# gortiz/pinot

Measured on AMD Instinct MI355X. Metric: rows scanned/sec + achieved HBM GB/s, filter+group-by query, 1/2/4/8 GPUs, higher is better.
Workload: dtype int32/int64/f64

## Files before the change

### include/pinot_amd.h

```cpp
#ifndef PINOT_AMD_H
#define PINOT_AMD_H

#include <stddef.h>
#include <stdint.h>

#ifdef __cplusplus
extern "C" {
#endif

#define PINOT_AMD_ABI_VERSION 1

#define PINOT_AMD_OK 0
#define PINOT_AMD_EINVAL (-1)
#define PINOT_AMD_EUNSUPPORTED (-2)
#define PINOT_AMD_EHIP (-3)
#define PINOT_AMD_ENOMEM (-4)
#define PINOT_AMD_EOVERFLOW (-5)

enum pinot_amd_data_type { PINOT_AMD_INT = 0, PINOT_AMD_LONG = 1, PINOT_AMD_FLOAT = 2, PINOT_AMD_DOUBLE = 3,
                           PINOT_AMD_STRING = 4 };

enum pinot_amd_fwd_encoding {
  PINOT_AMD_FWD_FIXED_BIT = 0,
  PINOT_AMD_FWD_RAW = 1,
// ... 121 lines not shown
int pinot_amd_result_accumulators(pinot_amd_result* r, int32_t* h_num_slots, int64_t* h_num_key_slots,
                                  void** h_slot_ptrs, int32_t* h_slot_ops);
int pinot_amd_result_export_groups(pinot_amd_result* r, uint64_t* d_keys, uint64_t* d_acc, int64_t cap,
                                   int32_t* h_key_words, int32_t* h_num_acc, int64_t* h_num_groups, void* stream);
int pinot_amd_result_merge_groups(pinot_amd_result* r, const uint64_t* d_keys, const uint64_t* d_acc, int64_t n,
                                  void* stream);
int pinot_amd_result_fetch_distinct_values(pinot_amd_result* r, int32_t agg_index, int64_t cap, int64_t* h_offsets,
                                           int64_t* h_values, int64_t* h_num_values);
int pinot_amd_result_fetch_value_counts(pinot_amd_result* r, int32_t agg_index, int64_t cap, int64_t* h_offsets,
                                        int64_t* h_values, int64_t* h_counts, int64_t* h_num_values);
const char* pinot_amd_result_distinct_string(pinot_amd_result* r, int32_t agg_index, int64_t id);

const char* pinot_amd_result_kernel_info(pinot_amd_result* r);
int pinot_amd_result_algorithmic_bytes(pinot_amd_result* r, double* h_bytes);
const char* pinot_amd_result_packed_info(pinot_amd_result* r);
const char* pinot_amd_result_plan_timing(pinot_amd_result* r);
int pinot_amd_result_last_kernel_ms(pinot_amd_result* r, double* h_ms);

#ifdef __cplusplus
}
#endif
#endif
```

### pinot_amd/_lib.py

```python
from __future__ import annotations

import ctypes as C
import os

try:
    import torch
except Exception:
    torch = None

HERE = os.path.dirname(os.path.abspath(__file__))
LIB_PATH = os.path.join(HERE, "libpinot_amd.so")


class PinotAmdError(RuntimeError):
    pass


class ColumnSpec(C.Structure):
    _fields_ = [
        ("name", C.c_char_p), ("stored_type", C.c_int32), ("encoding", C.c_int32), ("cardinality", C.c_int32),
        ("bits_per_element", C.c_int32), ("h_fwd", C.c_void_p), ("fwd_size", C.c_size_t),
        ("h_dictionary", C.c_void_p), ("dictionary_size", C.c_size_t), ("h_inverted", C.c_void_p),
        ("inverted_size", C.c_size_t),
    ]
# ... 65 lines not shown
    "pinot_amd_result_accumulators": (C.c_int, [_P, C.POINTER(C.c_int32), _I64P, _PP, C.POINTER(C.c_int32)]),
    "pinot_amd_result_check_word": (C.c_int, [_P, _PP]),
    "pinot_amd_selfcheck_failures": (C.c_int64, []),
    "pinot_amd_result_export_groups": (C.c_int, [_P, _P, _P, C.c_int64, C.POINTER(C.c_int32), C.POINTER(C.c_int32),
                                                 _I64P, _P]),
    "pinot_amd_result_merge_groups": (C.c_int, [_P, _P, _P, C.c_int64, _P]),
    "pinot_amd_result_plan_timing": (C.c_char_p, [_P]),
    "pinot_amd_query_set_result_limit": (C.c_int, [_P, C.c_int64, C.c_int64, C.c_int64]),
    "pinot_amd_query_add_order_by": (C.c_int, [_P, C.c_int32, C.c_int32, C.c_int32]),
    "pinot_amd_query_set_server_options": (C.c_int, [_P, C.c_int32, C.c_int64]),
    "pinot_amd_query_set_segment_trim": (C.c_int, [_P, C.c_int64]),
    "pinot_amd_result_last_kernel_ms": (C.c_int, [_P, C.POINTER(C.c_double)]),
    "pinot_amd_result_kernel_info": (C.c_char_p, [_P]),
    "pinot_amd_result_algorithmic_bytes": (C.c_int, [_P, C.POINTER(C.c_double)]),
    "pinot_amd_result_packed_info": (C.c_char_p, [_P]),
}

_lib = None


def lib():
    global _lib
    if _lib is None:
        if not os.path.exists(LIB_PATH):
            raise PinotAmdError(f"{LIB_PATH} not built: run `python -m pinot_amd.build` (no CPU fallback exists)")
        L = C.CDLL(LIB_PATH)
        for name, (res, args) in SIGNATURES.items():
            f = getattr(L, name)
            f.restype = res
            f.argtypes = args
# ... 9 lines not shown
```

### pinot_amd/csrc/device_types.h

```cpp
#pragma once
#include <stdint.h>

namespace pamd {

constexpr int kBlock = 256;
constexpr int kDocsPerThread = 4;
constexpr int kTileDocs = kBlock * kDocsPerThread;
constexpr int kMaxSlots = 16;
constexpr int kMaxLeaves = 16;
constexpr int kMaxClauses = 16;
constexpr int kMaxAcc = 16;
constexpr int kMaxGroupCols = 16;
constexpr int kMaxKeyWords = 8;
constexpr int kValueScanBlocks = 1024;
constexpr int kPadBytes = 4 * kTileDocs * 8 + 256;

enum : int32_t { ENC_FIXED_BIT = 0, ENC_RAW = 1, ENC_SORTED = 2 };
enum : int32_t { T_INT = 0, T_LONG = 1, T_FLOAT = 2, T_DOUBLE = 3, T_STRING = 4 };

enum : int32_t {
  LEAF_DICT_RANGE = 0,
  LEAF_DICT_SET = 1,
  LEAF_RAW_RANGE_I = 2,
  LEAF_RAW_RANGE_F = 3,
// ... 134 lines not shown
  unsigned long long* sel_entries;
  unsigned long long* sel_count;
  int64_t sel_cap;
  int32_t sel_chunk;
  int32_t sel_pad;
  const uint32_t* admit;
  int64_t admit_words;
  uint32_t* first;
  uint32_t* seen;
  unsigned long long* seen_n;
  int64_t seen_cap;
  unsigned long long* admit_flag;
  const unsigned long long* seg_cut;
  unsigned long long* seg_bits;
  int64_t seg_words;
};

}
```

### pinot_amd/csrc/host.cpp

```cpp
#include <dlfcn.h>
#include <hip/hip_runtime.h>

#include <algorithm>
#include <atomic>
#include <chrono>
#include <cmath>
#include <cstdarg>
#include <cstdio>
#include <cstdlib>
#include <cstring>
#include <deque>
#include <climits>
#include <limits>
#include <map>
#include <set>
#include <memory>
#include <mutex>
#include <string>
#include <new>
#include <stdexcept>
#include <thread>
#include <tuple>
#include <unordered_map>
#include <vector>
// ... 109 lines not shown
  do {                                                                                            \
    hipError_t e_ = (expr);                                                                       \
    if (e_ != hipSuccess) return fail(PINOT_AMD_EHIP, "%s: %s", #expr, hipGetErrorString(e_));   \
  } while (0)

namespace {

static const std::set<std::string>& kept_knobs() {
  static const std::set<std::string> kept = {
      "PINOT_AMD_ADMIT_PREFIX",
      "PINOT_AMD_ADMIT_SEQ",
      "PINOT_AMD_ATOMIC_HANDOVER",
      "PINOT_AMD_FILTER_GATE",
      "PINOT_AMD_FLUSH_EVERY",
      "PINOT_AMD_FLUSH_GROUP",
      "PINOT_AMD_FUSED_INV_SELECT",
      "PINOT_AMD_GENERIC_BITS",
      "PINOT_AMD_GROUP_PLAN",
      "PINOT_AMD_HASH_CAP_CACHE",
      "PINOT_AMD_HASH_DIRECT",
      "PINOT_AMD_HASH_INIT_SLOTS",
      "PINOT_AMD_HASH_LDS",
      "PINOT_AMD_HASH_LDS_ADMIT",
      "PINOT_AMD_HASH_LDS_SLOTS",
      "PINOT_AMD_HASH_MAX_PROBE",
      "PINOT_AMD_HASH_SPILL",
      "PINOT_AMD_HASH_TABLE_BYTES",
      "PINOT_AMD_INV_POLICY",
      "PINOT_AMD_NARROW_SUMS",
      "PINOT_AMD_PACKED",
// ... 1319 lines not shown
  std::vector<int32_t> agg_child;
  DevBuf bkeys;
  int64_t nbase = 0;
  ~DistinctFold();
};

struct pinot_amd_result {
  std::unique_ptr<DistinctFold> dc;
  hipStream_t stream = nullptr;
  PlanKind kind = PLAN_DENSE;
  DevQuery q{};
  std::deque<Launch> launches;
  std::vector<std::unique_ptr<DevBuf>> owned;
  bool filter_gate = false;
  std::vector<std::string> slot_names;
  struct InvLeaf {
    int seg;
    const Column* col;
    DevBuf* bitset;
    DevBuf* sel;
    DevBuf* grp;
    int32_t nsel, nchunks;
    int64_t num_docs;
    double alg_bytes;
    double bitset_bytes;
    DevBuf* psel = nullptr;
  };
  std::vector<InvLeaf> inv_leaves;
  DevBuf d_expand_jobs;
  int64_t expand_total = 0;
// ... 1900 lines not shown
        const __int128 b = c.vmin < 0 ? -(__int128)c.vmin : (__int128)c.vmin;
        m = std::max(m, std::max(a, b));
      }
      return m;
    };
    for (JitAcc& a : base.accs) {
      a.narrow = 0;
      if (a.op != ACC_SUM_I128 || env_is("PINOT_AMD_NARROW_SUMS", "0")) continue;
      __int128 m = maxabs(a.slot);
      if (m >= 0 && a.expr != EXPR_COL) {
        const __int128 m2 = maxabs(a.slot2);
        m = m2 < 0 ? -1 : a.expr == EXPR_MUL ? m * m2 : m + m2;
      }
      a.narrow = (m >= 0 && m * docs_bound <= (__int128)INT64_MAX) ? 1 : 0;
    }
  };
  auto lds_arrays = [&]() {
    int k = 0;
    jit_lds_layout(base, &k);
    return (int64_t)k;
  };
  int64_t lds_bytes = (int64_t)q.nacc * std::max<int64_t>(num_keys, 1) * 8;
  int64_t hash_lds_bytes = 0;
  std::vector<int64_t> part_vbase;
  if (r->kind == PLAN_DENSE && q.nacc > 0) {
    const int64_t min_grid = std::max<int64_t>(1, std::min<int64_t>(cus, all_tiles / kPartSub));
    set_narrow((__int128)((all_tiles + min_grid - 1) / min_grid) * kTileDocs);
    lds_bytes = lds_arrays() * std::max<int64_t>(num_keys, 1) * 8;
    if (lds_bytes <= 40 * 1024) {
      base.lds = true;
    } else if (lds_bytes <= lds_max && !env_is("PINOT_AMD_WIDE_LDS", "0")) {
      base.lds = true;
      base.scan_nsub = kPartSub;
    } else if (!env_is("PINOT_AMD_PARTITIONED", "0") && !Q.group_by.empty()) {
// ... 360 lines not shown
        if (m >= 0 && a.expr != EXPR_COL) {
          const __int128 m2 = maxabs(a.slot2);
          m = m2 < 0 ? -1 : a.expr == EXPR_MUL ? m * m2 : m + m2;
        }
        if (m >= 0 && m * (__int128)std::max<int64_t>(all_docs, 1) <= (__int128)INT64_MAX) {
          a.hbm_narrow = 1;
          arrs.push_back((int32_t)ai + 1);
        }
      }
    }
    r->n_sext = (int32_t)arrs.size();
    r->d_sext.reset();
    if (!arrs.empty())
      if (int rc = r->d_sext.alloc_copy(arrs.data(), arrs.size() * 4, 0)) return rc;
  }
  const size_t nl = r->launches.size();
  if (int rc = r->matched.alloc((3 * nl + 3) * sizeof(unsigned long long))) return rc;
  HIP_OK(hipMemset(r->matched.p, 0, r->matched.n));
  size_t max_count_cells = 0, max_rec = 0, max_slab = 0, max_slab_docs = 0;
  int64_t max_sel = 0;
  for (size_t li = 0; li < nl; ++li) {
    Launch& L = r->launches[li];
    std::vector<DevSegment> ls;
    std::vector<uint64_t*> lbits;
    int64_t tiles = 0;
    for (int si : L.segs) {
      DevSegment ds = hsegs[si];
      ds.tile_begin = tiles;
      ds.key_seg = r->admit ? si : key_seg[si];
      ds.pad = r->admit ? 1 : 0;
// ... 127 lines not shown
               : js.enc == ENC_RAW    ? value_size(js.type) : 0.0;
      }
      jp.depth = bpr <= 0 ? 1 : (int)std::min(4.0, std::max(1.0, std::ceil(4096.0 / (256.0 * bpr))));
      if (jp.sel_group > 1) jp.depth = std::max(1, (jp.depth + jp.sel_group - 1) / jp.sel_group);
      if (const char* pd = knob("PINOT_AMD_PREFETCH")) jp.depth = std::max(1, std::min(8, atoi(pd)));
      if (env_is("PINOT_AMD_LANE_TABLES", "0")) {
        for (auto& js : jp.slots) js.dict_regs = 0;
        for (auto& jl : jp.leaves) jl.bits_regs = 0;
      }
      if (const char* pw = knob("PINOT_AMD_WAVES_PER_EU")) jp.waves_per_eu = std::max(0, std::min(8, atoi(pw)));
      jp.nt_loads = env_is("PINOT_AMD_NT_LOADS", "1") ||
                    (!env_is("PINOT_AMD_NT_LOADS", "0") && bpr >= 15.0 && !jp.partitioned && !jp.select);
      jp.xcd_remap = env_is("PINOT_AMD_XCD_REMAP", "1") || (jp.admit && !env_is("PINOT_AMD_XCD_REMAP", "0"));
#ifdef PINOT_AMD_DIAGNOSTICS
      jp.diag_admit_off = env_is("PINOT_AMD_DIAG_ADMIT_OFF", "1");
      if (jp.partitioned) {
        const int64_t w = env_i64("PINOT_AMD_DIAG_REC_WRAP", 0);
        jp.diag_rec_wrap = (w >= 4096 && (w & (w - 1)) == 0) ? w : 0;
      }
#endif
    }
    if (jp.partitioned) {
      jit_layout_records(&jp);
      const int64_t stride = env_i64("PINOT_AMD_SAMPLE_STRIDE", 32);
      jp.part_sampled = stride > 0 && tiles >= 64 * stride && !env_is("PINOT_AMD_PART_SAMPLED", "0");
      if (jp.part_sampled) L.part.sample_stride = stride;
      jp.part_sub = (int)env_i64("PINOT_AMD_PART_SUB", kPartSub);
      if (jp.part_sub != 1 && jp.part_sub != 2) jp.part_sub = kPartSub;
      const size_t stage_lds = (size_t)lds_max / (size_t)(kPartSub / jp.part_sub);
      jp.admit_lds = jp.admit && jp.part_sub == kPartSub && !env_is("PINOT_AMD_ADMIT_LDS", "0") &&
// ... 819 lines not shown
  info.clear();
  for (size_t li = 0; li < r->launches.size(); ++li) {
    const Launch& L = r->launches[li];
    if (li) info += ";";
    bool first = true;
    for (size_t sl = 0; sl < r->slot_names.size() && !L.h_segs.empty(); ++sl) {
      if (!(L.packed >> sl & 1u)) continue;
      const DevColumn& dc = L.h_segs[0].cols[sl];
      info += (first ? "" : ",") + r->slot_names[sl] + ":" + std::to_string(dc.for_lo_bits) + "+" + std::to_string(dc.for_hi_bits);
      first = false;
    }
  }
  if (info.find_first_not_of(';') == std::string::npos) info.clear();
  return info.c_str();
}

static std::string kernel_info_of(pinot_amd_result* r) {
  std::string info;
  switch (r->kind) {
    case PLAN_PARTITIONED: info = "jit-partitioned"; break;
    case PLAN_HASH: info = r->trim ? "jit-hash-trim" : "jit-hash"; break;
    default: info = "jit";
  }
  if (r->kind == PLAN_HASH && r->hash_mode > 0) info += r->direct_ran ? "+direct" : "+nolds";
  for (const auto& L : r->launches)
    if (L.select) {
      info += L.fused ? "-fwselect" : L.word_select ? "-wselect" : "-select";
      break;
    }
  if (r->filter_gate) info += "+fgate";
// ... 886 lines not shown
```

### pinot_amd/csrc/jit.cpp

```cpp
#include <dlfcn.h>
#include <hip/hip_runtime.h>

#include <algorithm>
#include <cstdio>
#include <cstdlib>
#include <cstring>
#include <functional>
#include <map>
#include <mutex>
#include <sys/stat.h>
#include <unistd.h>
#include <sstream>
#include <numeric>
#include <string>
#include <vector>

#include "device_types.h"
#include "jit.h"
#include "jit_sources.inc"

namespace pamd {

namespace {

// ... 263 lines not shown
    case EXPR_MUL: return "(1.0 * (double)" + a + " * (double)" + b + ")";
    case EXPR_SUB: return "((double)" + a + " - (double)" + b + ")";
    default: return "(0.0 + (double)" + a + " + (double)" + b + ")";
  }
}

std::string acc_i64(const JitPlan& p, const JitAcc& A, const std::string& k) {
  return "(int64_t)" + value_expr(p, A.val(), k);
}
std::string acc_f64(const JitPlan& p, const JitAcc& A, const std::string& k) {
  return "(double)" + value_expr(p, A.val(), k);
}

}

std::vector<int> jit_lds_layout(const JitPlan& p, int* narrays) {
  std::vector<int> m(1 + p.accs.size(), 0);
  int k = 1;
  for (size_t a = 0; a < p.accs.size(); ++a) {
    const bool skip = p.accs[a].op == ACC_HI && a > 0 && p.accs[a - 1].op == ACC_SUM_I128 && p.accs[a - 1].narrow;
    m[a + 1] = skip ? -1 : k++;
  }
  if (narrays) *narrays = k;
  return m;
}

namespace {

std::string acc_off(const JitPlan& p, int i, bool lds = false, const std::string& stride = "") {
  if (!stride.empty()) {
    if (lds) i = jit_lds_layout(p, nullptr)[i];
    return "(int64_t)" + std::to_string(i) + " * " + stride;
  }
  if (p.hash) return "(int64_t)" + std::to_string(i) + " * H.cap";
  if (lds) i = jit_lds_layout(p, nullptr)[i];
  return std::to_string((int64_t)i * p.num_keys);
}

void emit_doc_acc(Emitter& e, const JitPlan& p, const std::string& ind, bool lds = false, const std::string& stride = "",
                  bool narrow = true) {
  e << ind << "add_u64(row, 1ull);\n";
  for (size_t a = 0; a < p.accs.size(); ++a) {
    const JitAcc& A = p.accs[a];
    if (A.op == ACC_HI) continue;
    const std::string o = "row + " + acc_off(p, (int)a + 1, lds, stride);
    switch (A.op) {
      case ACC_SUM_I64:
        e << ind << "add_u64(" << o << ", (uint64_t)(" << acc_i64(p, A, "k") << "));\n";
        break;
      case ACC_SUM_I128:
        if ((A.narrow && narrow) || (A.hbm_narrow && !lds))
          e << ind << "add_u64(" << o << ", (uint64_t)(" << acc_i64(p, A, "k") << "));\n";
        else
          e << ind << "{ const int64_t v = " << acc_i64(p, A, "k") << "; add128(" << o << ", row + "
            << acc_off(p, (int)a + 2, lds, stride) << ", (uint64_t)v, sext_hi(v)); }\n";
        break;
      case ACC_HI:
        break;
      case ACC_SUM_F64:
        e << ind << "add_f64(" << o << ", " << acc_f64(p, A, "k") << ");\n";
        break;
      case ACC_MIN:
        e << ind << "{ const double d = " << acc_f64(p, A, "k") << "; if (d == d) min_u64(" << o << ", ordered(d)); }\n";
        break;
      case ACC_MAX:
        e << ind << "{ const double d = " << acc_f64(p, A, "k") << "; if (d == d) max_u64(" << o << ", ordered(d)); }\n";
        break;
      default:
        e << ind << "min_u64(" << o << ", (uint64_t)(doc0 + k));\n";
        break;
    }
  }
}

void emit_block_count(Emitter& e, const std::string& out, int nthreads, const std::string& dyn = "") {
  if (nthreads == 64) {
    e << "  { const int64_t wm = wsum_i64(matched); if (lane == 0 && wm) atomicAdd(" << out << ", (unsigned long long)wm); }\n";
    return;
  }
  if (!dyn.empty())
    e << "  { __syncthreads();  // every wave is past its last table lookup\n"
// ... 1 lines not shown
  else
    e << "  { __shared__ unsigned long long blk_m_;\n";
  e << "    if (tid == 0) blk_m_ = 0ull;\n"
    << "    __syncthreads();\n"
    << "    const int64_t wm = wsum_i64(matched);\n"
    << "    if (lane == 0 && wm) atomicAdd(&blk_m_, (unsigned long long)wm);\n"
    << "    __syncthreads();\n"
    << "    if (tid == 0 && blk_m_) atomicAdd(" << out << ", blk_m_); }\n";
}

void emit_lds_flush(Emitter& e, const JitPlan& p, const std::string& ind, const std::string& src, int64_t src_keys,
                    const std::string& dst, int64_t dst_keys, const std::string& g_src, const std::string& g_dst) {
  const std::vector<int> lay = jit_lds_layout(p, nullptr);
  auto S = [&](int i) { return src + "[" + std::to_string((int64_t)lay[i] * src_keys) + " + " + g_src + "]"; };
  auto D = [&](int i) { return dst + " + " + std::to_string((int64_t)i * dst_keys) + " + " + g_dst; };
  e << ind << "add_u64(" << D(0) << ", " << S(0) << ");\n";
  for (size_t a = 0; a < p.accs.size(); ++a) {
    const int i = (int)a + 1;
    switch (p.accs[a].op) {
      case ACC_SUM_I64: e << ind << "add_u64(" << D(i) << ", " << S(i) << ");\n"; break;
      case ACC_SUM_I128:
        if (p.accs[a].hbm_narrow)
          e << ind << "add_u64(" << D(i) << ", " << S(i) << ");\n";
        else if (p.accs[a].narrow)
          e << ind << "add128(" << D(i) << ", " << D(i + 1) << ", " << S(i) << ", sext_hi((int64_t)" << S(i) << "));\n";
        else
          e << ind << "add128(" << D(i) << ", " << D(i + 1) << ", " << S(i) << ", " << S(i + 1) << ");\n";
        break;
      case ACC_HI: break;
      case ACC_SUM_F64: e << ind << "add_f64(" << D(i) << ", __longlong_as_double((long long)" << S(i) << "));\n"; break;
      case ACC_MAX: e << ind << "max_u64(" << D(i) << ", " << S(i) << ");\n"; break;
      default: e << ind << "min_u64(" << D(i) << ", " << S(i) << ");\n"; break;
    }
// ... 7 lines not shown
  std::ostringstream k;
  k << "v2|ns" << p.slots.size() << "|";
  for (auto& s : p.slots) {
    k << s.enc << "." << s.type << "." << s.bits << "." << s.dict_regs;
    if (s.packed) k << ".f" << s.for_lo << "." << s.for_hi;
    k << ",";
  }
  k << "|L";
  for (auto& l : p.leaves)
    k << l.slot << "." << l.clause << "." << l.negate << "." << l.kinds << "." << l.bits_regs << "." << l.lds_words << "."
      << l.mask << "." << l.lut << ",";
  k << "|c" << p.nclauses << "|G";
  for (auto& g : p.group) k << g.first << "." << g.second << ",";
  k << "|r" << p.any_remap << "|A";
  for (auto& a : p.accs)
    k << a.op << "." << a.slot << "." << a.expr << "." << a.slot2 << "." << a.nan_skip << "." << a.narrow << "." << a.hbm_narrow << ",";
  k << "|adm" << p.admit << "." << p.firstdoc << "." << p.admitseq << "." << p.diag_admit_off << "." << p.admit_lds << "."
    << p.diag_rec_wrap
    << "|x" << p.xcd_remap << "|fg" << p.filter_gate;
  k << "|so" << p.segpres << ":";
  for (auto& o : p.seg_ord) k << o.stride << "." << o.size << "." << o.ostride << "." << o.flip << ",";
  k << "|hl" << p.hash_lds << "." << p.hash_spill << "." << p.hash_admit << "." << p.hash_direct << "." << p.hash_probes;
  k << "|sel" << p.select << "." << p.word_select << "." << p.wsel_words << "." << p.sel_group << "|nk" << p.num_keys << "|lds" << p.lds << "." << p.scan_nsub << "|ag" << p.atomic_gate << "." << p.part_sampled << "|smp" << p.sample << "|d" << p.depth << "|w" << p.waves_per_eu << "|nt" << p.nt_loads << "|bs" << p.bitset << "|agg" << p.aggregate;
  if (p.hash) {
    k << "|H" << p.hash_words << "." << p.hash_seg << ":";
    for (auto& hp : p.hash_pack) k << hp.first << "." << hp.second << ",";
  }
  if (p.partitioned) {
    k << "|P" << p.nparts << "." << p.key_shift << "." << p.stage_cap << "." << p.part_sampled << "." << p.flush_pct << "."
      << p.flush_every << "." << p.flush_par << "." << p.flush_group << "." << p.part_sub << "." << p.scatter_batch << "|V";
    for (size_t j = 0; j < p.vals.size(); ++j)
      k << p.vals[j].expr << "." << p.vals[j].slot << "." << p.vals[j].slot2 << "."
        << (j < p.val_bits.size() ? p.val_bits[j] : -1) << ",";
// ... 364 lines not shown
          else if (p.accs[a].narrow)
            e << "    add128(" << D << ", row + (int64_t)" << i + 1 << " * H.cap, " << Sv << ", sext_hi((int64_t)" << Sv
              << "));\n";
          else
            e << "    add128(" << D << ", row + (int64_t)" << i + 1 << " * H.cap, " << Sv << ", LHA[" << (int64_t)lay[i + 1] * S
              << " + ls_]);\n";
          break;
        case ACC_HI: break;
        case ACC_SUM_F64: e << "    add_f64(" << D << ", __longlong_as_double((long long)" << Sv << "));\n"; break;
        case ACC_MAX: e << "    max_u64(" << D << ", " << Sv << ");\n"; break;
        default: e << "    min_u64(" << D << ", " << Sv << ");\n"; break;
      }
    }
    e << "  }\n";
  }
}

void emit_aggregate(Emitter& e, const JitPlan& p) {
  if (p.group.empty()) {
    e << "    RA0 += (int64_t)__builtin_popcount(match);\n";
    for (size_t a = 0; a < p.accs.size(); ++a) {
      const JitAcc& A = p.accs[a];
      const std::string r = "RA" + std::to_string(a + 1);
      switch (A.op) {
        case ACC_SUM_I64:
          e << "    for (int k = 0; k < 4; ++k) if ((match >> k) & 1u) " << r << " += " << acc_i64(p, A, "k") << ";\n";
          break;
        case ACC_SUM_I128:
          e << "    for (int k = 0; k < 4; ++k) if ((match >> k) & 1u) acc128(" << r << ", RA" << a + 2 << ", "
            << acc_i64(p, A, "k") << ");\n";
// ... 101 lines not shown
        << "      if (ls_ >= 0) {\n"
        << "        uint64_t* row = LHA + ls_;\n";
      emit_doc_acc(e, p, "        ", true, std::to_string(p.hash_lds), true);
      e << "        continue;\n      }\n";
    }
    e << "      const int64_t slot = hash_find<" << NW << ">(H, kw);\n"
      << "      if (slot < 0) { atomicAdd(H.overflow, 1ull); continue; }\n"
      << "      uint64_t* row = table + slot;\n";
    emit_doc_acc(e, p, "      ", false, "", false);
    e << "    }\n";
  } else {
    emit_group_key(e, p);
    emit_admit(e, p);
    emit_segtrim(e, p);
    e << "    const bool lane_has = match != 0u;\n"
      << "    const uint32_t kA = K[lane_has ? __builtin_ctz(match) : 0];\n"
      << "    bool lane_uniform = true;\n"
      << "    for (int k = 0; k < 4; ++k) lane_uniform &= !((match >> k) & 1u) || K[k] == kA;\n"
      << "    const unsigned long long has_mask = __ballot(lane_has);\n"
      << "    if (has_mask != 0ull) {\n"
      << "    const uint32_t kW = __shfl(kA, __ffsll((long long)has_mask) - 1, 64);\n"
      << "    if (__popcll(has_mask) >= 8 && __ballot(lane_has && (!lane_uniform || kA != kW)) == 0ull) {\n"
      << "      uint64_t* row = table + kW;\n"
      << "      { const int64_t c = wsum_i64(__builtin_popcount(match)); if (lane == 0) add_u64(row, (uint64_t)c); }\n";
    const std::vector<int> lay = jit_lds_layout(p, nullptr);
    for (size_t a = 0; a < p.accs.size(); ++a) {
      const JitAcc& A = p.accs[a];
      const int64_t off = (int64_t)(p.lds ? lay[a + 1] : (int)a + 1) * p.num_keys;
      switch (A.op) {
        case ACC_SUM_I64:
          e << "      { int64_t x = 0; for (int k = 0; k < 4; ++k) if ((match >> k) & 1u) x += " << acc_i64(p, A, "k")
            << "; x = wsum_i64(x); if (lane == 0) add_u64(row + " << off << ", (uint64_t)x); }\n";
          break;
        case ACC_SUM_F64:
          e << "      { double x = 0.0; for (int k = 0; k < 4; ++k) if ((match >> k) & 1u) x += " << acc_f64(p, A, "k")
            << "; x = wsum_f64(x); if (lane == 0) add_f64(row + " << off << ", x); }\n";
          break;
        case ACC_SUM_I128:
          if (A.narrow)
            e << "      { int64_t x = 0; for (int k = 0; k < 4; ++k) if ((match >> k) & 1u) x += " << acc_i64(p, A, "k")
              << "; x = wsum_i64(x); if (lane == 0) add_u64(row + " << off << ", (uint64_t)x); }\n";
          else
            e << "      { uint64_t lo = 0ull, hi = 0ull; for (int k = 0; k < 4; ++k) if ((match >> k) & 1u) acc128(lo, hi, "
// ... 11 lines not shown
            << "; const uint64_t o = ordered(d); if (((match >> k) & 1u) && d == d && o < x) x = o; }\n"
            << "        x = wmin_u64(x); if (lane == 0 && x != ~0ull) min_u64(row + " << off << ", x); }\n";
          break;
        default:
          e << "      { uint64_t x = 0ull; for (int k = 0; k < 4; ++k) { const double d = " << acc_f64(p, A, "k")
            << "; const uint64_t o = ordered(d); if (((match >> k) & 1u) && d == d && o > x) x = o; }\n"
            << "        x = wmax_u64(x); if (lane == 0 && x != 0ull) max_u64(row + " << off << ", x); }\n";
          break;
      }
    }
    e << "    } else {\n"
      << "      for (int k = 0; k < 4; ++k) {\n"
      << "        if (!((match >> k) & 1u)) continue;\n"
      << "        uint64_t* row = table + K[k];\n";
    emit_doc_acc(e, p, "        ", p.lds);
    e << "      }\n    }\n    }\n";
  }
}

std::string gen_scan(const JitPlan& p, int mode, const char* name, int nsub) {
  Emitter e;
  const int ns = (int)p.slots.size();
  const bool agg = p.aggregate && mode == MODE_SCAN;
  const int nthreads = 256 * nsub;
  const int P = p.nparts;
  const bool sample = mode == MODE_SAMPLE || mode == MODE_PSAMPLE;
  const bool pcount = mode == MODE_PCOUNT || mode == MODE_PSAMPLE;
  const bool psampled = p.partitioned && p.part_sampled;
  std::vector<bool> live(ns, !pcount && !sample && mode != MODE_SELECT && mode != MODE_FIRSTDOC &&
                                 mode != MODE_ADMITSEQ && mode != MODE_SEGPRES);
  for (auto& l : p.leaves)
// ... 135 lines not shown
      << "  (void)lds_stage; (void)wv;\n"
      << "  uint32_t PRD = 0u, OVC = 0u; (void)OVC;\n";
    if (p.admit && p.admit_lds)
      e << "  uint32_t* const ABL = (uint32_t*)((unsigned char*)lds_cur + " << scatter_admit_off(p, p.stage_cap) << ");\n"
        << "  int ABS = -1, ABW = 0;  // segment whose admission bitmap ABL holds; the block-uniform segment walker\n";
    e << "  for (int i = tid; i < " << P << "; i += " << nthreads << ") {\n";
    if (psampled)
      e << "    lds_cur[i] = (unsigned long long)part.offs[(int64_t)i * gridDim.x + bx];\n"
        << "    lds_end[i] = (unsigned long long)part.offs[(int64_t)i * gridDim.x + bx + 1];\n";
    else
      e << "    lds_cur[i] = (unsigned long long)(part.part_begin[i] + part.offs[(int64_t)i * gridDim.x * "
        << kPartCountRatio << " + (int64_t)bx * " << kPartCountRatio << "]);\n";
    e << "    lds_fill[i] = 0u;\n  }\n"
      << "  __syncthreads();\n";
  }
  const int64_t adm_words = (p.num_keys + 31) / 32;
  if (mode == MODE_ADMITSEQ) {
    e << "  extern __shared__ __attribute__((aligned(16))) uint32_t lds_adm[];\n"
      << "  uint32_t* const ABM = lds_adm;\n"
      << "  uint32_t* const AHK = lds_adm + " << adm_words << ";\n"
      << "  uint32_t* const AHD = AHK + " << kAdmitSeqSlots << ";\n"
      << "  uint32_t* const AHL = AHD + " << kAdmitSeqSlots << ";  // slots the tile inserted\n"
      << "  uint32_t* const AMS = AHL + " << kTileDocs << ";\n"
      << "  for (int i = tid; i < " << adm_words << "; i += " << nthreads << ") ABM[i] = 0u;\n"
      << "  for (int i = tid; i < " << kAdmitSeqSlots << "; i += " << nthreads << ") { AHK[i] = 0xFFFFFFFFu; AHD[i] = 0xFFFFFFFFu; }\n"
      << "  for (int i = tid; i < 80; i += " << nthreads << ") AMS[i] = 0u;\n"
      << "  __syncthreads();\n"
      << "  long long ACNT = 0;  // distinct keys the segment holds so far (block-uniform)\n"
      << "  bool ADONE = false;\n"
      << "  int APAR = 0;\n";
// ... 427 lines not shown
      << "      for (int i = tid; i < (int)tnew; i += " << nthreads << ") {\n"
      << "        const uint32_t sl = AHL[i], o = AHD[sl] - tdoc0;\n"
      << "        const uint32_t r = AMS[34 + (o >> 5)] + __popc(AMS[2 + (o >> 5)] & ((1u << (o & 31u)) - 1u));\n"
      << "        if ((long long)r < need) atomicOr(&ABM[AHK[sl] >> 5], 1u << (AHK[sl] & 31u));\n"
      << "      }\n"
      << "      ADONE = true;\n"
      << "    } else {\n"
      << "      for (int i = tid; i < (int)tnew; i += " << nthreads << ") {\n"
      << "        const uint32_t sl = AHL[i], kk = AHK[sl];\n"
      << "        atomicOr(&ABM[kk >> 5], 1u << (kk & 31u)); AHK[sl] = 0xFFFFFFFFu; AHD[sl] = 0xFFFFFFFFu;\n"
      << "      }\n"
      << "      ACNT += tnew;\n"
      << "    }\n"
      << "    __syncthreads();\n";
  }
  if (agg) emit_aggregate(e, p);
  e << "    }\n";
  };
  auto emit_gate_mask = [&](const std::string& st, const std::string& out, const std::string& segi, const std::string& tile) {
    const std::string fs = "f" + st.substr(1);
    e << "    { const PJ_C DevSegment& seg = segs[" << segi << "];\n"
      << "      const int64_t tdoc_ = (" << tile << " - seg.tile_begin) * " << kTileDocs << ";\n"
      << "      const int64_t doc0 = tdoc_ + (int64_t)ltid * 4;\n"
      << "      const int32_t rem_ = (" << tile << ") < t_end ? (int32_t)min(seg.num_docs - tdoc_, (int64_t)" << kTileDocs << ") : 0;\n"
      << "      uint32_t match = 0xFu >> min(max(ltid * 4 + 4 - rem_, 0), 4);\n";
    for (int sl = 0; sl < ns; ++sl)
      if (gate_slot[sl]) emit_decode(e, p.slots[sl], sl, fs);
    emit_reloads(segi);
    emit_filter(fs, false);
    e << "      " << out << " = match;\n    }\n";
  };
// ... 575 lines not shown
  for (auto& a : p.accs) {
    if (a.op == ACC_FIRST_DOC) continue;
    live[a.slot] = true;
    if (a.expr != EXPR_COL) live[a.slot2] = true;
  }
  const int nthreads = p.lds ? 256 * p.scan_nsub : 256;
  e << "extern \"C\" __global__ void __launch_bounds__(" << nthreads << ") pinot_gather(const DevSegment* __restrict__ segs_in,\n"
    << "    const DevQuery q, uint64_t* __restrict__ acc, uint64_t* const* __restrict__ bitset_out,\n"
    << "    unsigned long long* __restrict__ matched_out, const DevPartition part, const DevHash H) {\n"
    << "  using namespace pjit;\n"
    << "  const PJ_C DevSegment* segs = (const PJ_C DevSegment*)segs_in;\n"
    << "  const int tid = threadIdx.x, lane = tid & 63;\n";
  if (p.lds) emit_lds_table_init(e, p, nthreads);
  else e << "  uint64_t* const table = acc;\n";
  if (p.group.empty()) emit_agg_registers(e, p);
  e << "  const unsigned long long nent = min(q.sel_count[0], (unsigned long long)q.sel_cap);\n"
    << "  const int64_t nquads = (int64_t)(nent >> 2);\n"
    << "  const PJ_G uint4* ent = (const PJ_G uint4*)q.sel_entries;\n"
    << "  for (int64_t q0 = (int64_t)blockIdx.x * " << nthreads << "; q0 < nquads; q0 += (int64_t)gridDim.x * " << nthreads << ") {\n"
    << "    const int64_t qi = q0 + tid;\n"
    << "    uint32_t pend = 0u, vmask = 0u, mseg = 0u;\n"
    << "    int64_t DK[4] = {0, 0, 0, 0};\n"
    << "    if (qi < nquads) {\n"
    << "      const uint4 a = ent[2 * qi], b = ent[2 * qi + 1];\n"
    << "      const uint32_t dk[4] = {a.x, a.z, b.x, b.z};\n"
    << "      mseg = a.y;\n"
    << "      for (int k = 0; k < 4; ++k) { const bool v = dk[k] != 0xFFFFFFFFu; vmask |= (uint32_t)v << k; DK[k] = v ? (int64_t)dk[k] : 0; }\n"
    << "      pend = vmask != 0u ? 1u : 0u;  // a quad of padding reads nothing\n"
    << "    }\n"
    << "    while (true) {\n"
// ... 339 lines not shown
    plans.push_back(p);
    p.scan_nsub = 1;
    p.slots[0].bits = 9;
    const int shapes[][4] = {{0, 10, 32, 8}, {16, 8, 32, 16}, {16, 0, 32, 0}, {0, 0, 0, 16}, {0, 1, 16, 12}};
    for (auto& sh : shapes) {
      p.slots[1].packed = p.slots[2].packed = 1;
      p.slots[1].for_lo = sh[0], p.slots[1].for_hi = sh[1];
      p.slots[2].for_lo = sh[2], p.slots[2].for_hi = sh[3];
      p.filter_gate = false;
      p.nt_loads = true;
      plans.push_back(p);
      p.filter_gate = true;
      p.nt_loads = false;
      plans.push_back(p);
    }
  }
  {
    JitPlan p;
    p.slots = {{ENC_SORTED, T_INT}, {ENC_FIXED_BIT, T_DOUBLE}, {ENC_RAW, T_FLOAT}, {ENC_FIXED_BIT, T_LONG}};
    p.leaves = {{0, 0, 1, (1u << LEAF_DICT_SET) | (1u << LEAF_CONST) | (1u << LEAF_DOC_RANGE)},
                {2, 0, 0, 1u << LEAF_RAW_RANGE_F}, {2, 1, 1, 1u << LEAF_RAW_IN_F}, {-1, 1, 0, 1u << LEAF_DOC_BITSET}};
    p.nclauses = 2;
    p.group = {{0, 1}, {1, 50}};
    p.any_remap = true;
    p.accs = {{ACC_MIN, 1}, {ACC_SUM_F64, 2}, {ACC_SUM_I64, 3}, {ACC_MAX, 3}};
    p.num_keys = 5000000;
    p.lds = false;
    plans.push_back(p);
    p.filter_gate = true;
    plans.push_back(p);
// ... 414 lines not shown
```

### pinot_amd/csrc/jit.h

```cpp
#pragma once
#include <hip/hip_runtime.h>

#include <stdint.h>

#include <string>
#include <utility>
#include <vector>

namespace pamd {

constexpr int kPartSub = 4;
constexpr int kPartCountRatio = 2;
constexpr int64_t kAdmitSeqMaxKeys = 1 << 20;
constexpr int kAdmitSeqSlots = 2048;
constexpr int kHashLdsProbes = 8;
inline size_t jit_admitseq_lds(int64_t num_keys) {
  return (size_t)((num_keys + 31) / 32) * 4 + kAdmitSeqSlots * 8 + 1024 * 4 + 80 * 4;
}

struct JitSlot {
  int enc;
  int type;
  int bits = 0;
  int dict_regs = 0;
// ... 13 lines not shown
enum { EXPR_COL = 0, EXPR_MUL = 1, EXPR_SUB = 2, EXPR_ADD = 3 };
struct JitVal {
  int expr = EXPR_COL;
  int slot = 0;
  int slot2 = -1;
  bool operator==(const JitVal& o) const { return expr == o.expr && slot == o.slot && slot2 == o.slot2; }
};
struct JitAcc {
  int op;
  int slot;
  int expr = EXPR_COL;
  int slot2 = -1;
  int nan_skip = 0;
  int narrow = 0;
  int hbm_narrow = 0;
  JitVal val() const { return JitVal{expr, slot, slot2}; }
};
struct JitPlan {
  std::vector<JitSlot> slots;
  std::vector<JitLeaf> leaves;
  int nclauses = 0;
  std::vector<std::pair<int, int64_t>> group;
  bool any_remap = false;
  std::vector<JitAcc> accs;
  int64_t num_keys = 1;
  bool lds = false;
  int scan_nsub = 1;
  int depth = 1;
  int waves_per_eu = 0;
  bool nt_loads = false;
// ... 25 lines not shown
  bool hash_direct = false;
  bool select = false;
  bool admit = false;
  bool firstdoc = false;
  bool admit_lds = false;
  bool admitseq = false;
  bool word_select = false;
  int wsel_words = 4;
  int sel_group = 1;
  bool xcd_remap = false;
  bool filter_gate = false;
  int hash_admit = 0;
  int hash_probes = kHashLdsProbes;
  bool diag_admit_off = false;
  int64_t diag_rec_wrap = 0;
  struct OrdCol { int64_t stride, size, ostride; int flip; };
  std::vector<OrdCol> seg_ord;
  bool segpres = false;
};
void jit_layout_records(JitPlan* p);
int jit_val_natural_bits(const JitPlan& p, const JitVal& v);
bool jit_val_is_int(const JitPlan& p, const JitVal& v);
size_t jit_scatter_lds(const JitPlan& p, int cap);
std::vector<int> jit_lds_layout(const JitPlan& p, int* narrays);
struct JitKernel {
  std::vector<char> image;
  hipModule_t module = nullptr;
  hipFunction_t fn = nullptr;
  hipFunction_t fn_scatter = nullptr;
  hipFunction_t fn_agg = nullptr;
  hipFunction_t fn_ovf = nullptr;
  hipFunction_t fn_gather = nullptr;
};
const char* jit_val_ctype(const JitPlan& p, const JitVal& v);
int jit_val_size(const JitPlan& p, const JitVal& v);

std::string jit_shape_key(const JitPlan& p);
std::string jit_generate(const JitPlan& p);
std::string jit_full_source(const JitPlan& p);
// ... 4 lines not shown
```

### pinot_amd/engine.py

```python
from __future__ import annotations

import ctypes as C
import gc
import math
from typing import Dict, List, Optional, Sequence

import numpy as np

from . import _lib
from ._lib import ColumnSpec, PredicateSpec, check, lib
from .query import (VALUE_SET_FUNCS, DistinctSize, FinalValue, JavaDouble, QueryContext, fold_distinct_count,
                    hists_from_csr, parse_sql, reduce_rows, server_table, sets_from_csr, split_distinct_count)
from .segment import ColumnBuffers, SegmentBuffers, DOUBLE, FLOAT, INT, LONG, STRING

TYPE_CODE = {INT: 0, LONG: 1, FLOAT: 2, DOUBLE: 3, STRING: 4}
ENC_CODE = {"FIXED_BIT": 0, "RAW": 1, "SORTED": 2}
PRED_CODE = {"EQ": 0, "NOT_EQ": 1, "IN": 2, "NOT_IN": 3, "RANGE": 4}
AGG_CODE = {"COUNT": 0, "SUM": 1, "MIN": 2, "MAX": 3, "SUMLONG": 4, "AVG": 5, "MINMAXRANGE": 6,
            "DISTINCTCOUNT": 7, "PERCENTILE": 8, "DISTINCTSUM": 9, "DISTINCTAVG": 10}
EXPR_CODE = {"MUL": 1, "SUB": 2, "ADD": 3}


def _stream_handle(stream) -> Optional[int]:
    if stream is None:
# ... 207 lines not shown
        check(lib().pinot_amd_result_num_docs_matched(self._h, C.byref(out)), "num_docs_matched")
        return out.value

    def num_groups_limit_reached(self) -> bool:
        if self._merged_reached is not None:
            return self._merged_reached
        out = C.c_int32()
        check(lib().pinot_amd_result_num_groups_limit_reached(self._h, C.byref(out)), "num_groups_limit_reached")
        return bool(out.value)

    def kernel_info(self) -> str:
        return lib().pinot_amd_result_kernel_info(self._h).decode()

    def packed_info(self) -> str:
        return lib().pinot_amd_result_packed_info(self._h).decode()

    def last_kernel_ms(self) -> float:
        out = C.c_double()
        check(lib().pinot_amd_result_last_kernel_ms(self._h, C.byref(out)), "last_kernel_ms")
        return out.value

    def plan_timing(self) -> Dict[str, float]:
        txt = lib().pinot_amd_result_plan_timing(self._h).decode()
        return {k: float(v) for k, v in (kv.split("=") for kv in txt.split(";") if kv)}

    def algorithmic_bytes(self) -> float:
        out = C.c_double()
        check(lib().pinot_amd_result_algorithmic_bytes(self._h, C.byref(out)), "algorithmic_bytes")
        return out.value

# ... 347 lines not shown
```

Before: 403.6 billion.

## Pack count and narrow integer sums into one LDS word per group

```diff
diff --git a/include/pinot_amd.h b/include/pinot_amd.h
--- a/include/pinot_amd.h
+++ b/include/pinot_amd.h
@@ -159,6 +159,7 @@
 const char* pinot_amd_result_kernel_info(pinot_amd_result* r);
 int pinot_amd_result_algorithmic_bytes(pinot_amd_result* r, double* h_bytes);
 const char* pinot_amd_result_packed_info(pinot_amd_result* r);
+const char* pinot_amd_result_fused_info(pinot_amd_result* r);
 const char* pinot_amd_result_plan_timing(pinot_amd_result* r);
 int pinot_amd_result_last_kernel_ms(pinot_amd_result* r, double* h_ms);
 
diff --git a/pinot_amd/_lib.py b/pinot_amd/_lib.py
--- a/pinot_amd/_lib.py
+++ b/pinot_amd/_lib.py
@@ -103,6 +103,7 @@
     "pinot_amd_result_kernel_info": (C.c_char_p, [_P]),
     "pinot_amd_result_algorithmic_bytes": (C.c_int, [_P, C.POINTER(C.c_double)]),
     "pinot_amd_result_packed_info": (C.c_char_p, [_P]),
+    "pinot_amd_result_fused_info": (C.c_char_p, [_P]),
 }
 
 _lib = None
diff --git a/pinot_amd/csrc/device_types.h b/pinot_amd/csrc/device_types.h
--- a/pinot_amd/csrc/device_types.h
+++ b/pinot_amd/csrc/device_types.h
@@ -172,6 +172,7 @@
   const unsigned long long* seg_cut;
   unsigned long long* seg_bits;
   int64_t seg_words;
+  int64_t fuse_lo[kMaxAcc];
 };
 
 }
diff --git a/pinot_amd/csrc/host.cpp b/pinot_amd/csrc/host.cpp
--- a/pinot_amd/csrc/host.cpp
+++ b/pinot_amd/csrc/host.cpp
@@ -147,6 +147,7 @@
       "PINOT_AMD_FILTER_GATE",
       "PINOT_AMD_FLUSH_EVERY",
       "PINOT_AMD_FLUSH_GROUP",
+      "PINOT_AMD_FUSED_ACC",
       "PINOT_AMD_FUSED_INV_SELECT",
       "PINOT_AMD_GENERIC_BITS",
       "PINOT_AMD_GROUP_PLAN",
@@ -1496,6 +1497,7 @@
   std::vector<std::unique_ptr<DevBuf>> owned;
   bool filter_gate = false;
   std::vector<std::string> slot_names;
+  std::string fused_info;
   struct InvLeaf {
     int seg;
     const Column* col;
@@ -3426,10 +3428,42 @@
       }
       a.narrow = (m >= 0 && m * docs_bound <= (__int128)INT64_MAX) ? 1 : 0;
     }
+    auto bitlen = [](unsigned __int128 w) {
+      int b = 0;
+      for (; w; w >>= 1) ++b;
+      return b;
+    };
+    int shift = bitlen((unsigned __int128)std::max<__int128>(docs_bound, 1));
+    for (size_t ai = 0; ai < base.accs.size(); ++ai) {
+      JitAcc& a = base.accs[ai];
+      a.fused = a.fuse_shift = a.fuse_bits = 0;
+      q.fuse_lo[ai + 1] = 0;
+      if (!a.narrow || a.expr != EXPR_COL || Q.group_by.empty() || env_is("PINOT_AMD_FUSED_ACC", "0")) continue;
+      bool any = false, known = true;
+      int64_t lo = 0, hi = 0;
+      for (auto* s : segs) {
+        const Column& c = *s->cols.at(slot_cols[a.slot]);
+        if (s->num_docs == 0) continue;
+        if (!c.has_range) { known = false; break; }
+        lo = any ? std::min(lo, c.vmin) : c.vmin;
+        hi = any ? std::max(hi, c.vmax) : c.vmax;
+        any = true;
+      }
+      if (!known) continue;
+      const int fb = bitlen((unsigned __int128)((__int128)hi - (__int128)lo) * (unsigned __int128)std::max<__int128>(docs_bound, 1));
+      if (shift + fb > 64) continue;
+      a.fused = 1;
+      a.fuse_shift = shift;
+      a.fuse_bits = fb;
+      q.fuse_lo[ai + 1] = lo;
+      shift += fb;
+    }
   };
   auto lds_arrays = [&]() {
+    JitPlan t = base;
+    for (JitAcc& a : t.accs) a.fused = 0;
     int k = 0;
-    jit_lds_layout(base, &k);
+    jit_lds_layout(t, &k);
     return (int64_t)k;
   };
   int64_t lds_bytes = (int64_t)q.nacc * std::max<int64_t>(num_keys, 1) * 8;
@@ -3820,6 +3854,12 @@
     if (!arrs.empty())
       if (int rc = r->d_sext.alloc_copy(arrs.data(), arrs.size() * 4, 0)) return rc;
   }
+  r->fused_info.clear();
+  for (const JitAcc& a : base.accs) {
+    if (!jit_acc_fused(base, a)) continue;
+    if (r->fused_info.empty()) r->fused_info = "count:" + std::to_string(a.fuse_shift);
+    r->fused_info += "," + slot_cols[a.slot] + ":" + std::to_string(a.fuse_shift) + "+" + std::to_string(a.fuse_bits);
+  }
   const size_t nl = r->launches.size();
   if (int rc = r->matched.alloc((3 * nl + 3) * sizeof(unsigned long long))) return rc;
   HIP_OK(hipMemset(r->matched.p, 0, r->matched.n));
@@ -3977,6 +4017,7 @@
       jp.xcd_remap = env_is("PINOT_AMD_XCD_REMAP", "1") || (jp.admit && !env_is("PINOT_AMD_XCD_REMAP", "0"));
 #ifdef PINOT_AMD_DIAGNOSTICS
       jp.diag_admit_off = env_is("PINOT_AMD_DIAG_ADMIT_OFF", "1");
+      jp.diag_no_agg = env_is("PINOT_AMD_DIAG_NO_AGG", "1");
       if (jp.partitioned) {
         const int64_t w = env_i64("PINOT_AMD_DIAG_REC_WRAP", 0);
         jp.diag_rec_wrap = (w >= 4096 && (w & (w - 1)) == 0) ? w : 0;
@@ -4826,6 +4867,8 @@
   if (info.find_first_not_of(';') == std::string::npos) info.clear();
   return info.c_str();
 }
+
+const char* pinot_amd_result_fused_info(pinot_amd_result* r) { return r ? r->fused_info.c_str() : ""; }
 
 static std::string kernel_info_of(pinot_amd_result* r) {
   std::string info;
diff --git a/pinot_amd/csrc/jit.cpp b/pinot_amd/csrc/jit.cpp
--- a/pinot_amd/csrc/jit.cpp
+++ b/pinot_amd/csrc/jit.cpp
@@ -301,11 +301,16 @@
 
 }
 
+bool jit_acc_fused(const JitPlan& p, const JitAcc& A) {
+  return p.lds && !p.hash && !p.partitioned && !p.group.empty() && A.op == ACC_SUM_I128 && A.narrow && A.fused;
+}
+
 std::vector<int> jit_lds_layout(const JitPlan& p, int* narrays) {
   std::vector<int> m(1 + p.accs.size(), 0);
   int k = 1;
   for (size_t a = 0; a < p.accs.size(); ++a) {
-    const bool skip = p.accs[a].op == ACC_HI && a > 0 && p.accs[a - 1].op == ACC_SUM_I128 && p.accs[a - 1].narrow;
+    const bool skip = (p.accs[a].op == ACC_HI && a > 0 && p.accs[a - 1].op == ACC_SUM_I128 && p.accs[a - 1].narrow) ||
+                      jit_acc_fused(p, p.accs[a]);
     m[a + 1] = skip ? -1 : k++;
   }
   if (narrays) *narrays = k;
@@ -326,10 +331,20 @@
 
 void emit_doc_acc(Emitter& e, const JitPlan& p, const std::string& ind, bool lds = false, const std::string& stride = "",
                   bool narrow = true) {
-  e << ind << "add_u64(row, 1ull);\n";
+  const bool fuse = lds && stride.empty() && narrow;
+  e << ind << "add_u64(row, 1ull";
+  for (size_t a = 0; fuse && a < p.accs.size(); ++a) {
+    const JitAcc& A = p.accs[a];
+    if (!jit_acc_fused(p, A) || A.fuse_bits == 0) continue;
+    if (jit_val_size(p, A.val()) == 4)
+      e << " | ((uint64_t)((uint32_t)" << value_expr(p, A.val(), "k") << " - (uint32_t)FLO" << a + 1 << ") << " << A.fuse_shift << ")";
+    else
+      e << " | (((uint64_t)(" << acc_i64(p, A, "k") << ") - FLO" << a + 1 << ") << " << A.fuse_shift << ")";
+  }
+  e << ");\n";
   for (size_t a = 0; a < p.accs.size(); ++a) {
     const JitAcc& A = p.accs[a];
-    if (A.op == ACC_HI) continue;
+    if (A.op == ACC_HI || (fuse && jit_acc_fused(p, A))) continue;
     const std::string o = "row + " + acc_off(p, (int)a + 1, lds, stride);
     switch (A.op) {
       case ACC_SUM_I64:
@@ -348,10 +363,10 @@
         e << ind << "add_f64(" << o << ", " << acc_f64(p, A, "k") << ");\n";
         break;
       case ACC_MIN:
-        e << ind << "{ const double d = " << acc_f64(p, A, "k") << "; if (d == d) min_u64(" << o << ", ordered(d)); }\n";
+        e << ind << "{ const double d = " << acc_f64(p, A, "k") << "; min_u64(" << o << ", d == d ? ordered(d) : ~0ull); }\n";
         break;
       case ACC_MAX:
-        e << ind << "{ const double d = " << acc_f64(p, A, "k") << "; if (d == d) max_u64(" << o << ", ordered(d)); }\n";
+        e << ind << "{ const double d = " << acc_f64(p, A, "k") << "; max_u64(" << o << ", d == d ? ordered(d) : 0ull); }\n";
         break;
       default:
         e << ind << "min_u64(" << o << ", (uint64_t)(doc0 + k));\n";
@@ -383,9 +398,27 @@
   const std::vector<int> lay = jit_lds_layout(p, nullptr);
   auto S = [&](int i) { return src + "[" + std::to_string((int64_t)lay[i] * src_keys) + " + " + g_src + "]"; };
   auto D = [&](int i) { return dst + " + " + std::to_string((int64_t)i * dst_keys) + " + " + g_dst; };
-  e << ind << "add_u64(" << D(0) << ", " << S(0) << ");\n";
+  int cbits = 64;
+  for (const JitAcc& A : p.accs)
+    if (jit_acc_fused(p, A)) cbits = std::min(cbits, A.fuse_shift);
+  if (cbits < 64) {
+    e << ind << "const uint64_t w_ = " << S(0) << ", c_ = w_ & " << ((1ull << cbits) - 1) << "ull;\n"
+      << ind << "add_u64(" << D(0) << ", c_);\n";
+  } else {
+    e << ind << "add_u64(" << D(0) << ", " << S(0) << ");\n";
+  }
   for (size_t a = 0; a < p.accs.size(); ++a) {
     const int i = (int)a + 1;
+    if (jit_acc_fused(p, p.accs[a])) {
+      const JitAcc& A = p.accs[a];
+      const std::string f = A.fuse_bits == 0 ? std::string("0ull")
+                            : "((w_ >> " + std::to_string(A.fuse_shift) + ")" +
+                              (A.fuse_shift + A.fuse_bits < 64 ? " & " + std::to_string((1ull << A.fuse_bits) - 1) + "ull" : std::string()) + ")";
+      e << ind << "{ const uint64_t s_ = " << f << " + c_ * FLO" << i << ";\n";
+      if (A.hbm_narrow) e << ind << "  add_u64(" << D(i) << ", s_); }\n";
+      else e << ind << "  add128(" << D(i) << ", " << D(i + 1) << ", s_, sext_hi((int64_t)s_)); }\n";
+      continue;
+    }
     switch (p.accs[a].op) {
       case ACC_SUM_I64: e << ind << "add_u64(" << D(i) << ", " << S(i) << ");\n"; break;
       case ACC_SUM_I128:
@@ -423,9 +456,10 @@
   for (auto& g : p.group) k << g.first << "." << g.second << ",";
   k << "|r" << p.any_remap << "|A";
   for (auto& a : p.accs)
-    k << a.op << "." << a.slot << "." << a.expr << "." << a.slot2 << "." << a.nan_skip << "." << a.narrow << "." << a.hbm_narrow << ",";
+    k << a.op << "." << a.slot << "." << a.expr << "." << a.slot2 << "." << a.nan_skip << "." << a.narrow << "." << a.hbm_narrow
+      << "." << a.fused << "." << a.fuse_shift << "." << a.fuse_bits << ",";
   k << "|adm" << p.admit << "." << p.firstdoc << "." << p.admitseq << "." << p.diag_admit_off << "." << p.admit_lds << "."
-    << p.diag_rec_wrap
+    << p.diag_rec_wrap << "." << p.diag_no_agg
     << "|x" << p.xcd_remap << "|fg" << p.filter_gate;
   k << "|so" << p.segpres << ":";
   for (auto& o : p.seg_ord) k << o.stride << "." << o.size << "." << o.ostride << "." << o.flip << ",";
@@ -820,6 +854,13 @@
     }
     e << "  }\n";
   }
+}
+
+constexpr int kUniformSkipMax = 16;
+void emit_uniform_state(Emitter& e, const JitPlan& p) {
+  if (!p.group.empty() && !p.hash) e << "  int UFS = 0, UFP = 0;  // tiles left to skip the test, the current penalty\n";
+  for (size_t a = 0; a < p.accs.size(); ++a)
+    if (jit_acc_fused(p, p.accs[a])) e << "  const uint64_t FLO" << a + 1 << " = (uint64_t)q.fuse_lo[" << a + 1 << "];\n";
 }
 
 void emit_aggregate(Emitter& e, const JitPlan& p) {
@@ -951,19 +992,35 @@
     emit_admit(e, p);
     emit_segtrim(e, p);
     e << "    const bool lane_has = match != 0u;\n"
-      << "    const uint32_t kA = K[lane_has ? __builtin_ctz(match) : 0];\n"
-      << "    bool lane_uniform = true;\n"
-      << "    for (int k = 0; k < 4; ++k) lane_uniform &= !((match >> k) & 1u) || K[k] == kA;\n"
-      << "    const unsigned long long has_mask = __ballot(lane_has);\n"
-      << "    if (has_mask != 0ull) {\n"
-      << "    const uint32_t kW = __shfl(kA, __ffsll((long long)has_mask) - 1, 64);\n"
-      << "    if (__popcll(has_mask) >= 8 && __ballot(lane_has && (!lane_uniform || kA != kW)) == 0ull) {\n"
+      << "    bool wave_uniform = false;\n"
+      << "    uint32_t kW = 0u;\n"
+      << "    if (UFS > 0) {\n"
+      << "      --UFS;\n"
+      << "    } else {\n"
+      << "      const unsigned long long has_mask = __ballot(lane_has);\n"
+      << "      if (has_mask != 0ull) {\n"
+      << "        const uint32_t kA = K[lane_has ? __builtin_ctz(match) : 0];\n"
+      << "        bool lane_uniform = true;\n"
+      << "        for (int k = 0; k < 4; ++k) lane_uniform &= !((match >> k) & 1u) || K[k] == kA;\n"
+      << "        kW = (uint32_t)__builtin_amdgcn_readlane((int)kA, __ffsll((long long)has_mask) - 1);\n"
+      << "        wave_uniform = __popcll(has_mask) >= 8 && __ballot(lane_has && (!lane_uniform || kA != kW)) == 0ull;\n"
+      << "        if (wave_uniform) { UFP = 0; } else { UFP = UFP ? min(2 * UFP, " << kUniformSkipMax << ") : 1; UFS = UFP; }\n"
+      << "      }\n"
+      << "    }\n"
+      << "    if (wave_uniform) {\n"
       << "      uint64_t* row = table + kW;\n"
-      << "      { const int64_t c = wsum_i64(__builtin_popcount(match)); if (lane == 0) add_u64(row, (uint64_t)c); }\n";
+      << "      { const int64_t c = wsum_i64(__builtin_popcount(match));\n"
+      << "        uint64_t w0 = (uint64_t)c;\n";
+    for (size_t a = 0; a < p.accs.size(); ++a)
+      if (jit_acc_fused(p, p.accs[a]) && p.accs[a].fuse_bits > 0)
+        e << "        { int64_t x = 0; for (int k = 0; k < 4; ++k) if ((match >> k) & 1u) x += " << acc_i64(p, p.accs[a], "k")
+          << "; x = wsum_i64(x); w0 |= ((uint64_t)x - (uint64_t)c * FLO" << a + 1 << ") << " << p.accs[a].fuse_shift << "; }\n";
+    e << "        if (lane == 0) add_u64(row, w0); }\n";
     const std::vector<int> lay = jit_lds_layout(p, nullptr);
     for (size_t a = 0; a < p.accs.size(); ++a) {
       const JitAcc& A = p.accs[a];
       const int64_t off = (int64_t)(p.lds ? lay[a + 1] : (int)a + 1) * p.num_keys;
+      if (jit_acc_fused(p, A)) continue;
       switch (A.op) {
         case ACC_SUM_I64:
           e << "      { int64_t x = 0; for (int k = 0; k < 4; ++k) if ((match >> k) & 1u) x += " << acc_i64(p, A, "k")
@@ -1005,7 +1062,7 @@
       << "        if (!((match >> k) & 1u)) continue;\n"
       << "        uint64_t* row = table + K[k];\n";
     emit_doc_acc(e, p, "        ", p.lds);
-    e << "      }\n    }\n    }\n";
+    e << "      }\n    }\n";
   }
 }
 
@@ -1171,6 +1228,7 @@
     e << "    lds_fill[i] = 0u;\n  }\n"
       << "  __syncthreads();\n";
   }
+  if (agg) emit_uniform_state(e, p);
   const int64_t adm_words = (p.num_keys + 31) / 32;
   if (mode == MODE_ADMITSEQ) {
     e << "  extern __shared__ __attribute__((aligned(16))) uint32_t lds_adm[];\n"
@@ -1628,7 +1686,19 @@
       << "    }\n"
       << "    __syncthreads();\n";
   }
-  if (agg) emit_aggregate(e, p);
+  if (agg && p.diag_no_agg && !p.group.empty() && !p.hash) {
+    emit_group_key(e, p);
+    e << "    for (int k = 0; k < 4; ++k) asm volatile(\"\" :: \"v\"(K[k]));\n";
+    for (const JitAcc& A : p.accs) {
+      if (A.op == ACC_HI || A.op == ACC_FIRST_DOC) continue;
+      const bool f = A.op == ACC_SUM_F64 || A.op == ACC_MIN || A.op == ACC_MAX;
+      e << "    for (int k = 0; k < 4; ++k) { const uint64_t x_ = (uint64_t)"
+        << (f ? "__double_as_longlong(" + acc_f64(p, A, "k") + ")" : "(" + acc_i64(p, A, "k") + ")")
+        << "; asm volatile(\"\" :: \"v\"((uint32_t)x_), \"v\"((uint32_t)(x_ >> 32))); }\n";
+    }
+  } else if (agg) {
+    emit_aggregate(e, p);
+  }
   e << "    }\n";
   };
   auto emit_gate_mask = [&](const std::string& st, const std::string& out, const std::string& segi, const std::string& tile) {
@@ -2234,6 +2304,7 @@
   if (p.lds) emit_lds_table_init(e, p, nthreads);
   else e << "  uint64_t* const table = acc;\n";
   if (p.group.empty()) emit_agg_registers(e, p);
+  emit_uniform_state(e, p);
   e << "  const unsigned long long nent = min(q.sel_count[0], (unsigned long long)q.sel_cap);\n"
     << "  const int64_t nquads = (int64_t)(nent >> 2);\n"
     << "  const PJ_G uint4* ent = (const PJ_G uint4*)q.sel_entries;\n"
@@ -2603,6 +2674,15 @@
       p.nt_loads = false;
       plans.push_back(p);
     }
+    p.filter_gate = false;
+    p.nt_loads = true;
+    p.accs[0].fused = 1, p.accs[0].fuse_shift = 22, p.accs[0].fuse_bits = 32;
+    plans.push_back(p);
+    p.accs[2].fused = 1, p.accs[2].fuse_shift = 54, p.accs[2].fuse_bits = 10;
+    plans.push_back(p);
+    p.accs[2].fuse_bits = 0;
+    p.scan_nsub = 4;
+    plans.push_back(p);
   }
   {
     JitPlan p;
diff --git a/pinot_amd/csrc/jit.h b/pinot_amd/csrc/jit.h
--- a/pinot_amd/csrc/jit.h
+++ b/pinot_amd/csrc/jit.h
@@ -51,6 +51,7 @@
   int nan_skip = 0;
   int narrow = 0;
   int hbm_narrow = 0;
+  int fused = 0, fuse_shift = 0, fuse_bits = 0;
   JitVal val() const { return JitVal{expr, slot, slot2}; }
 };
 struct JitPlan {
@@ -106,6 +107,7 @@
   int hash_probes = kHashLdsProbes;
   bool diag_admit_off = false;
   int64_t diag_rec_wrap = 0;
+  bool diag_no_agg = false;
   struct OrdCol { int64_t stride, size, ostride; int flip; };
   std::vector<OrdCol> seg_ord;
   bool segpres = false;
@@ -115,6 +117,7 @@
 bool jit_val_is_int(const JitPlan& p, const JitVal& v);
 size_t jit_scatter_lds(const JitPlan& p, int cap);
 std::vector<int> jit_lds_layout(const JitPlan& p, int* narrays);
+bool jit_acc_fused(const JitPlan& p, const JitAcc& A);
 struct JitKernel {
   std::vector<char> image;
   hipModule_t module = nullptr;
diff --git a/pinot_amd/engine.py b/pinot_amd/engine.py
--- a/pinot_amd/engine.py
+++ b/pinot_amd/engine.py
@@ -245,6 +245,9 @@
 
     def packed_info(self) -> str:
         return lib().pinot_amd_result_packed_info(self._h).decode()
+
+    def fused_info(self) -> str:
+        return lib().pinot_amd_result_fused_info(self._h).decode()
 
     def last_kernel_ms(self) -> float:
         out = C.c_double()
```

Measured after the change: 406.8 billion (median of 6 runs). About the same (+0.8%).
